# Kangfei/NNGP-src

Measured on AMD Instinct MI355X. Metric: NNGP kernel-build + GP-solve wall-clock (ms) and GFLOP/s at N train queries, higher is better.
Workload: dtype f32 (Cholesky products as split f16 x3, f32 accumulate; f64 build/CG/means; the posterior's float64-grade residual as exact int8 digit-plane products); 1 GPU; synthetic N=32768, d=128, 5-layer ReLU NNGP + full Cholesky posterior (configs[2], north-star target); N=32768, d=128, n_relu=3, get=nngp, M_test=1024, parallelism=single GPU

## Files before the change

nngp-src_amd/csrc/api.hip:

```cpp
#include "model.h"

namespace nngp {

static thread_local char g_err[1024] = "";

void set_error(const char* fmt, ...) {
    va_list ap;
    va_start(ap, fmt);
    vsnprintf(g_err, sizeof(g_err), fmt, ap);
    va_end(ap);
}

int make_arch_dev(const nngp_arch* arch, ArchDev* out) {
    NNGP_REQUIRE(arch != nullptr, "arch is NULL");
    NNGP_REQUIRE(arch->n_dense >= 1 && arch->n_dense <= NNGP_MAX_DENSE, "arch.n_dense must be in [1, %d] (got %d)",
                 NNGP_MAX_DENSE, arch->n_dense);
    out->n_dense = arch->n_dense;
    for (int l = 0; l < NNGP_MAX_DENSE; ++l) {
        out->w2[l] = l < arch->n_dense ? arch->w_std[l] * arch->w_std[l] : 0.0;
        out->b2[l] = l < arch->n_dense ? arch->b_std[l] * arch->b_std[l] : 0.0;
    }
    return 0;
}

// ... 205 lines not shown
    int rc = 0;
    m->arch = *arch;
    m->n_cap = n_cap; m->np_cap = round_up(n_cap, TB); m->m_cap = 0;
    m->ld = m->np_cap;
    m->d = d; m->ny = ny; m->get = get; m->diag_reg = diag_reg; m->absolute = diag_reg_absolute_scale;
    const int64_t np = m->np_cap;
    auto A = [&](int r) { if (rc == 0) rc = r; };
    A(dev_alloc(&m->x, n_cap * d)); A(dev_alloc(&m->y, n_cap * ny)); A(dev_alloc(&m->q, n_cap));
    A(dev_alloc(&m->kdiag, n_cap)); A(dev_alloc(&m->k64, np * np)); A(dev_alloc(&m->a32, np * np));
    A(dev_alloc(&m->dinv, (np / TB) * TB * TB)); A(dev_alloc(&m->clamped, 1)); A(dev_alloc(&m->alpha, n_cap * ny));
    A(dev_alloc(&m->pcg.r, np)); A(dev_alloc(&m->pcg.z, np)); A(dev_alloc(&m->pcg.p, np)); A(dev_alloc(&m->pcg.q, np));
    A(dev_alloc(&m->pcg.xcol, np)); A(dev_alloc(&m->pcg.bcol, np));
    A(dev_alloc(&m->pcg.f32a, np)); A(dev_alloc(&m->pcg.f32b, np)); A(dev_alloc(&m->pcg.f32c, np));
    A(dev_alloc(&m->pcg.scal, 32));
    A(dev_alloc(&m->pcg.symv_part, (np / TB) * np));
    A(dev_alloc(&m->pcg.dot_part, 32));
    A(dev_alloc(&m->pcg.dot_ctr, 1));
    if (rc == 0 && hipMemset(m->pcg.dot_ctr, 0, sizeof(unsigned)) != hipSuccess) rc = -1;
    m->pcg.symv_np = np;
    {
        const int64_t bs_cap = triinv_block(np);
        const int64_t nblk = (np + bs_cap - 1) / bs_cap;
        A(dev_alloc(&m->tri.tinv, nblk * bs_cap * bs_cap)); A(dev_alloc(&m->tri.xinv, nblk * bs_cap * bs_cap));
        A(dev_alloc(&m->tri.partial, (bs_cap / TB) * np)); A(dev_alloc(&m->tri.tmp, bs_cap));
    }
    if (rc == 0 && hipHostMalloc(reinterpret_cast<void**>(&m->pcg.host_scal), sizeof(double) * 32) != hipSuccess) {
        set_error("model_create: hipHostMalloc failed");
        rc = -1;
    }
    if (rc == 0) rc = lookahead_create(&m->la);
    int prio_least = 0, prio_greatest = 0;
    if (hipDeviceGetStreamPriorityRange(&prio_least, &prio_greatest) != hipSuccess) prio_least = prio_greatest = 0;
    if (rc == 0 && (hipStreamCreateWithPriority(&m->solve_stream, hipStreamNonBlocking, prio_greatest) != hipSuccess ||
                    hipEventCreateWithFlags(&m->ev_ready, hipEventDisableTiming) != hipSuccess ||
                    hipEventCreateWithFlags(&m->ev_lt, hipEventDisableTiming) != hipSuccess ||
                    hipEventCreateWithFlags(&m->ev_solved, hipEventDisableTiming) != hipSuccess ||
                    hipEventCreateWithFlags(&m->ev_predict, hipEventDisableTiming) != hipSuccess)) {
        set_error("model_create: could not create the solve stream");
        rc = -1;
    }
    if (rc == 0 && np >= 4 * kLookAheadNb) {
        m->split.rows_cap = np + 256;
        m->split.k_cap = kLookAheadNb;
        m->split.col_stride = m->split.rows_cap * m->split.k_cap * 4;
        const int64_t ncols = (np + kLookAheadNb - 1) / kLookAheadNb;
        rc = dev_alloc(&m->split.planes, ncols * m->split.col_stride);
        if (rc == 0) rc = dev_alloc(&m->split.counters, 16);
// ... 149 lines not shown
}

int nngp_model_factor_input_rows(nngp_model* m, int64_t row_begin, int64_t row_end, double shift_scale, void* stream) {
    hipStream_t s = (hipStream_t)stream;
    NNGP_REQUIRE(m != nullptr && m->built, "factor_input_rows: build the kernel rows first");
    NNGP_REQUIRE(0 <= row_begin && row_begin <= row_end && row_end <= m->n && shift_scale >= 1.0, "factor_input_rows: bad row range or shift");
    NNGP_TRY(drop_pending_solve(m));
    m->reg_fac = m->reg * shift_scale;
    m->k64_partial = true;
    return launch_factor_input(m->k64, m->ld, m->a32, m->ld, m->n, m->np, m->reg_fac, m->reg_fac + m->trace_mean, s, row_begin, row_end);
}

int nngp_model_factor_input_complete(nngp_model* m) {
    NNGP_REQUIRE(m != nullptr && m->built, "factor_input_complete: build the kernel rows first");
    NNGP_REQUIRE(m->k64_partial, "factor_input_complete: no rows of the factor input were converted (nngp_model_factor_input_rows) since the last build");
    m->a32_complete = true;
    return 0;
}

int nngp_model_precond(nngp_model* m, const double* r, double* z, void* stream) {
    NNGP_REQUIRE(m != nullptr && m->factored, "precond: factor first");
    NNGP_REQUIRE(r != nullptr && z != nullptr, "precond: NULL argument");
    NNGP_TRY(tri_join(m, (hipStream_t)stream));
    return precond_apply(m->a32, m->ld, m->tri, m->n, m->np, r, z, m->pcg, (hipStream_t)stream);
}

int nngp_model_matvec_rows(nngp_model* m, const double* p, double* q, int64_t row_begin, int64_t row_end, void* stream) {
    NNGP_REQUIRE(m != nullptr && m->built, "matvec_rows: build the kernel rows first");
    NNGP_REQUIRE(p != nullptr && q != nullptr && 0 <= row_begin && row_begin <= row_end && row_end <= m->n, "matvec_rows: bad arguments");
    return launch_gemv_f64(m->k64 + row_begin * m->ld, m->ld, row_end - row_begin, m->n, p, 1, q, 1, 0.0, (hipStream_t)stream);
}

int nngp_model_set_alpha(nngp_model* m, const double* alpha, int32_t iters, double rel_residual, void* stream) {
    hipStream_t s = (hipStream_t)stream;
    NNGP_REQUIRE(m != nullptr && m->factored && alpha != nullptr, "set_alpha: factor first");
    NNGP_TRY(drop_pending_solve(m));
    NNGP_HIP_CHECK(hipMemcpyAsync(m->alpha, alpha, sizeof(double) * m->n * m->ny, hipMemcpyDeviceToDevice, s));
    m->solved = true;
    m->solve_pending = false;
    m->cg_partial = false;
    m->have_alpha_event = false;
    m->iters = iters;
    m->relres = rel_residual;
    return 0;
}

int nngp_model_factor_end(nngp_model* m, void* stream) {
    hipStream_t s = (hipStream_t)stream;
    NNGP_REQUIRE(m != nullptr && m->built, "factor_end: build the kernel rows first");
    m->tri.bs = triinv_block(m->np);
    m->tri_stale = true;
    m->tri_pending = false;
    if (!m->split.l_ready && m->split.planes != nullptr && m->np >= 4 * m->split.k_cap && m->tri.bs % m->split.k_cap == 0 &&
        m->split.rows_cap >= m->np + 256) {
        const int64_t bs = m->split.k_cap, ldp = 4 * bs;
        for (int64_t j = 0, o = 0; o + bs < m->np; ++j, o += bs)
            NNGP_TRY(launch_split_rows(m->a32 + (o + bs) * m->ld + o, m->ld, m->np - o - bs, bs, m->split.scale,
                                       m->split.planes + j * m->split.col_stride + (o + bs) * ldp, ldp, s));
        m->split.l_ready = true;
    }
    m->factored = true;
    m->solved = false;
    m->lt_ready = false;
    return 0;
}

int nngp_model_factor_buffers(nngp_model* m, float** a32, int64_t* ld, float** dinv) {
    NNGP_REQUIRE(m != nullptr && m->have_train, "factor_buffers: call set_train first");
    if (a32) *a32 = m->a32;
    if (ld) *ld = m->ld;
    if (dinv) *dinv = m->dinv;
    return 0;
}

int nngp_model_factor(nngp_model* m, void* stream) {
// ... 49 lines not shown
    m->serving_ready = false;
    m->i8.k.ready = false;
    m->i8_checked = m->i8_distrusted = false;
    m->i8_guard_pending = false;
    BuildArgs a{};
    a.x1 = m->x; a.x2 = m->x; a.q1 = m->q; a.q2 = m->q;
    a.n1 = n1; a.n2 = n1; a.d = m->d;
    a.row_begin = n0; a.row_end = n1; a.sym = 0;
    a.ld64 = a.ld32 = m->ld;
    if (m->get == NNGP_GET_NNGP) a.nngp64 = m->k64; else a.ntk64 = m->k64;
    m->k64_symmetric = false;
    NNGP_TRY(launch_kernel_build(a, m->arch, s));
    NNGP_TRY(launch_mirror_rows_f64(m->k64, m->ld, n0, n1, s));
    NNGP_TRY(launch_zero_pad_f64(m->k64, m->ld, n1, np1, s));
    NNGP_TRY(launch_factor_input(m->k64, m->ld, m->a32, m->ld, n1, np1, m->reg_fac, m->reg_fac + m->trace_mean, s, r0));
    float* a10 = m->a32 + r0 * m->ld;
    NNGP_TRY(tri_join(m, s));
    NNGP_TRY(trsm_rlt_blocks_f32(a10, m->ld, rows, m->a32, m->ld, m->tri, r0, m->trsm_tmp, s));
    NNGP_TRY(launch_gemm_nt_f32(a10 + r0, m->ld, a10, m->ld, a10, m->ld, rows, rows, r0, -1.0f, 1.0f, true, s));
    NNGP_TRY(potrf_f32(a10 + r0, rows, m->ld, m->dinv + (r0 / TB) * TB * TB, m->clamped, (float)(0.25 * m->reg_fac), s));
    m->tri.bs = triinv_block(m->np);
    m->tri_stale = true;
    m->tri_pending = false;
    NNGP_TRY(tri_join(m, s));
    if (m->split.l_ready && m->split.scale == old_scale && m->split.rows_cap >= np1 + 256) {
        const int64_t bs = m->split.k_cap, ldp = 4 * bs;
        for (int64_t j = 0, o = 0; o + bs < np1; ++j, o += bs) {
            const int64_t first = (o + bs > r0) ? o + bs : r0;
            NNGP_TRY(launch_split_rows(m->a32 + first * m->ld + o, m->ld, np1 - first, bs, m->split.scale,
                                       m->split.planes + j * m->split.col_stride + first * ldp, ldp, s));
        }
    } else {
        m->split.l_ready = false;
    }
    m->split.lt_ready = false;
    m->lt_ready = false;
    m->aux_ready = false;
    (void)np0;
    return 0;
}

constexpr int kSolveAhead = 6;

constexpr double kPartialTol = 1e-6;

static void note_solve(nngp_model* m, int it, double rr) {
    int est = it;
    if (rr > m->pend_tol && rr > 0.0 && rr < 1.0 && it > 0) est = (int)ceil(it * log(m->pend_tol) / log(rr));
    if (est > m->iters) m->iters = est;
    if (rr > m->relres) m->relres = rr;
}

}
namespace nngp {
int run_pending_solve(nngp_model* m, hipStream_t user, bool order_user, bool allow_partial) {
    hipStream_t s = m->solve_stream;
    auto join_tri = [&]() -> int {
        NNGP_HIP_CHECK(hipStreamWaitEvent(s, m->ev_ready, 0));
        return tri_join(m, s);
    };
    if (!m->solve_pending) {
        if (!m->cg_partial || allow_partial) {
            if (order_user && m->solved && m->have_alpha_event) NNGP_HIP_CHECK(hipStreamWaitEvent(user, m->ev_solved, 0));
            return 0;
        }
        if (m->have_predict_event) NNGP_HIP_CHECK(hipStreamWaitEvent(s, m->ev_predict, 0));
        int it = 0;
        double rr = 0.0;
        NNGP_TRY(join_tri());
        NNGP_TRY(pcg_finish(m->k64, m->ld, m->n, m->reg, m->a32, m->ld, m->tri, m->np, m->pcg.xcol, m->pcg, m->cg_iters_done,
                            m->pend_max_iters, m->pend_tol, &it, &rr, s, true));
        NNGP_TRY(launch_strided_copy_f64(m->pcg.xcol, 1, m->alpha, m->ny, m->n, s));
        m->cg_partial = false;
        m->iters = 0;
        m->relres = 0.0;
        note_solve(m, it, rr);
        NNGP_HIP_CHECK(hipEventRecord(m->ev_solved, s));
        m->have_alpha_event = true;
        if (order_user) NNGP_HIP_CHECK(hipStreamWaitEvent(user, m->ev_solved, 0));
        else NNGP_HIP_CHECK(hipStreamSynchronize(s));
        return 0;
    }
// ... 30 lines not shown
            note_solve(m, it, rr);
        }
    }
    NNGP_HIP_CHECK(hipEventRecord(m->ev_solved, s));
    m->have_alpha_event = true;
    if (order_user) NNGP_HIP_CHECK(hipStreamWaitEvent(user, m->ev_solved, 0));
    else NNGP_HIP_CHECK(hipStreamSynchronize(s));
    return 0;
}

}

extern "C" {

int nngp_model_solve(nngp_model* m, int32_t max_iters, double tol, void* stream) {
    hipStream_t s = (hipStream_t)stream;
    NNGP_REQUIRE(m != nullptr && m->factored, "solve: factor first");
    NNGP_REQUIRE(!m->k64_partial, "solve: this model holds only its own kernel rows (row-sharded layout): the caller drives the CG "
                                  "(nngp_model_precond, nngp_model_matvec_rows) and hands alpha back with nngp_model_set_alpha");
    NNGP_TRY(drop_pending_solve(m));
    const double weak = (m->reg > 0.0 && m->reg_fac > m->reg) ? sqrt(m->reg_fac / m->reg) : 1.0;
    m->pend_max_iters = max_iters > 0 ? max_iters : (int)fmin(2000.0, 60.0 * weak);
    m->pend_tol = tol > 0.0 ? tol : 1e-10;
    NNGP_HIP_CHECK(hipEventRecord(m->ev_ready, s));
    m->solve_pending = true;
    m->solved = true;
    if (NNGP_KNOB(7) == 3) return run_pending_solve(m, s, true);
    if (NNGP_KNOB(0) & 32) return run_pending_solve(m, s, true, true);
    if (m->ny == 1 && NNGP_KNOB(0) == 64) {
        const int ahead = m->pend_max_iters < kSolveAhead ? m->pend_max_iters : kSolveAhead;
        NNGP_HIP_CHECK(hipStreamWaitEvent(m->solve_stream, m->ev_ready, 0));
        NNGP_TRY(tri_join(m, m->solve_stream));
        NNGP_TRY(launch_strided_copy_f64(m->y, 1, m->pcg.bcol, 1, m->n, m->solve_stream));
        NNGP_TRY(pcg_begin(m->k64, m->ld, m->n, m->reg, m->a32, m->ld, m->tri, m->np, m->pcg.bcol, m->pcg.xcol, m->pcg, ahead,
                           m->solve_stream));
        m->solve_ahead = ahead;
    }
    return 0;
}

int nngp_model_fit(nngp_model* m, const double* x, const double* y, int64_t n, void* stream) {
    NNGP_TRY(nngp_model_set_train(m, x, y, n, stream));
    NNGP_TRY(nngp_model_build_rows(m, 0, n, stream));
    NNGP_TRY(nngp_model_factor(m, stream));
    return nngp_model_solve(m, 0, 0.0, stream);
}

int nngp_model_kernel_buffer(nngp_model* m, double** k64, int64_t* ld) {
    NNGP_REQUIRE(m != nullptr && m->have_train, "kernel_buffer: call set_train first");
    if (k64) *k64 = m->k64;
    if (ld) *ld = m->ld;
    return 0;
}

int nngp_model_update_timer(nngp_model* m, int32_t enable) {
// ... 142 lines not shown
```

nngp-src_amd/csrc/api_predict.hip:

```cpp
#include "model.h"

namespace nngp {

int ensure_predict_capacity(nngp_model* m, int64_t mt, bool need_ktd) {
    if (mt > m->m_cap || m->b32 == nullptr) {
        const int64_t cap = mt > m->m_cap ? mt : m->m_cap;
        NNGP_HIP_CHECK(hipDeviceSynchronize());
        dev_free(m->xt_q); dev_free(m->tt_diag); dev_free(m->b32); dev_free(m->trsm_tmp);
        NNGP_TRY(dev_alloc(&m->xt_q, cap));
        NNGP_TRY(dev_alloc(&m->tt_diag, cap));
        NNGP_TRY(dev_alloc(&m->b32, round_up(cap, TB) * m->np_cap));
        NNGP_TRY(dev_alloc(&m->trsm_tmp, round_up(cap, TB) * triinv_block(m->np_cap)));
        if (m->split.planes != nullptr) {
            dev_free(m->split.planes_b); dev_free(m->split.row_inv);
            m->split.planes_b = nullptr; m->split.row_inv = nullptr;
            m->split.mb_cap = round_up(cap, TB);
            m->split.b_panels = (int)((triinv_block(m->np_cap) + m->split.k_cap - 1) / m->split.k_cap);
            NNGP_TRY(dev_alloc(&m->split.planes_b, (int64_t)(m->split.b_panels - 1) * m->split.col_stride + (m->split.mb_cap + 256) * m->split.k_cap * 4));
            NNGP_TRY(dev_alloc(&m->split.row_inv, m->split.mb_cap));
            tk_destroy(m->tk);
            m->tk = nullptr;
            if (m->split.k_cap == 1024 && triinv_block(m->np_cap) == 1024) NNGP_TRY(tk_create(&m->tk, m->np_cap, m->split.mb_cap) < 0 ? -1 : 0);
        }
        m->m_cap = cap;
// ... 254 lines not shown
    }
    NNGP_TRY(launch_gemm_nt_f64(out, np, rhs, np, z, np, m->k64, m->ld, mp, np, np, -1.0, 1.0, s));
    return launch_axpby_mat(out, 1.0, z, -m->reg, np, mp, np, s);
}

int tri_join(nngp_model* m, hipStream_t s) {
    if (m->tri_stale) {
        if (m->ev_tri == nullptr) NNGP_HIP_CHECK(hipEventCreateWithFlags(&m->ev_tri, hipEventDisableTiming));
        NNGP_TRY(triinv_build(m->a32, m->ld, m->dinv, m->np, m->tri, s));
        if (m->tk != nullptr && m->tri.bs == 1024) NNGP_TRY(tk_prepare_inverses(m->tk, m->tri, m->np, m->a32, m->ld, s));
        NNGP_HIP_CHECK(hipEventRecord(m->ev_tri, s));
        m->tri_stale = false;
        m->tri_pending = true;
        return 0;
    }
    if (m->tri_pending) NNGP_HIP_CHECK(hipStreamWaitEvent(s, m->ev_tri, 0));
    if (m->tk != nullptr && !tk_inverses_ready(m->tk) && m->tri.bs == 1024) {
        NNGP_TRY(tk_prepare_inverses(m->tk, m->tri, m->np, m->a32, m->ld, s));
        if (m->ev_tri == nullptr) NNGP_HIP_CHECK(hipEventCreateWithFlags(&m->ev_tri, hipEventDisableTiming));
        NNGP_HIP_CHECK(hipEventRecord(m->ev_tri, s));
        m->tri_pending = true;
    }
    return 0;
}

int tri_fork(nngp_model* m, hipStream_t s) {
    if (!m->tri_stale || m->la == nullptr || m->la->panel == nullptr || NNGP_KNOB(5) == 61) return 0;
    if (m->ev_tri == nullptr) NNGP_HIP_CHECK(hipEventCreateWithFlags(&m->ev_tri, hipEventDisableTiming));
    if (m->ev_tri_fork == nullptr) NNGP_HIP_CHECK(hipEventCreateWithFlags(&m->ev_tri_fork, hipEventDisableTiming));
    NNGP_HIP_CHECK(hipEventRecord(m->ev_tri_fork, s));
    NNGP_HIP_CHECK(hipStreamWaitEvent(m->la->panel, m->ev_tri_fork, 0));
    NNGP_TRY(triinv_build(m->a32, m->ld, m->dinv, m->np, m->tri, m->la->panel));
    if (m->tk != nullptr && m->tri.bs == 1024) NNGP_TRY(tk_prepare_inverses(m->tk, m->tri, m->np, m->a32, m->ld, m->la->panel));
    NNGP_HIP_CHECK(hipEventRecord(m->ev_tri, m->la->panel));
    m->tri_stale = false;
    m->tri_pending = true;
    return 0;
}

bool use_split_solves(const nngp_model* m, int64_t mp) {
    return m->split.l_ready && m->split.planes_b != nullptr && mp <= m->split.mb_cap && m->tri.bs % m->split.k_cap == 0 &&
           m->tri.bs / m->split.k_cap <= m->split.b_panels && m->tri.bs <= 2048 && NNGP_KNOB(7) == 0 && mp >= 256 && mp * m->np >= 7000000;
}

bool use_tickets(const nngp_model* m, int64_t mp) {
    return !m->tk_failed && m->tri.bs == 1024 && tk_usable(m->tk, mp, m->np) && NNGP_KNOB(9) != 16;
// ... 534 lines not shown
```

nngp-src_amd/csrc/common.h:

```cpp
#pragma once
#include <hip/hip_runtime.h>
#include <stdint.h>
#include <atomic>
#include <stdio.h>
#include <string.h>

#include "../../include/nngp_hip.h"
#include "../../include/nngp_rbf_gp.h"
#include "../../include/nngp_activations.h"
#include "../../include/nngp_mll.h"

namespace nngp {

constexpr int TB = 128;

void set_error(const char* fmt, ...);
void note_alloc();
#ifdef NNGP_TIMING_KNOBS
extern std::atomic<int> g_knobs[16];
#define NNGP_KNOB(i) (nngp::g_knobs[i].load(std::memory_order_relaxed))
#else
#define NNGP_KNOB(i) 0
#endif

// ... 207 lines not shown
struct I8Fuse {
    float* out32 = nullptr;
    int64_t ld32 = 0;
    double* part = nullptr;
};
int64_t i8s_col_blocks(int64_t cols);
int launch_i8s_combine(double* out, int64_t ldo, const double* cin, int64_t ldcin, double beta, double alpha, const double* g,
                       int64_t ldg, double gamma, const int32_t* partial, int64_t ldc, int64_t slab, int nchunk, int ndiag,
                       const double* sa, const double* sb, int64_t rows, int64_t cols, hipStream_t s, const I8Fuse* fuse = nullptr);
int launch_i8s_rowstat_finish(const double* part, int64_t cols, int64_t rows, const double* base, double* var, double* delta,
                              double* zstat, hipStream_t s);

int launch_gemm_nt_f64(double* c, int64_t ldc, const double* cin, int64_t ldcin, const double* a, int64_t lda,
                       const double* b, int64_t ldb, int64_t m, int64_t n, int64_t k, double alpha, double beta,
                       hipStream_t s, int kmode = 0);

int launch_transpose_blocks_f32(const float* src, float* dst, int64_t bs, int64_t count, hipStream_t s);
struct TriInv {
    int64_t bs = 0;
    float* tinv = nullptr;
    float* xinv = nullptr;
    float* partial = nullptr;
    float* tmp = nullptr;
    int64_t done_blocks = 0;
};
int64_t triinv_block(int64_t np);
int triinv_build(const float* l, int64_t ld, const float* dinv, int64_t np, TriInv& ti, hipStream_t s);
int triinv_build_range(const float* l, int64_t ld, const float* dinv, int64_t np, TriInv& ti, int64_t j0, int64_t j1, hipStream_t s);
int trsm_rlt_blocks_f32(float* b, int64_t ldb, int64_t m, const float* l, int64_t ld, const TriInv& ti, int64_t np,
                        float* tmp, hipStream_t s);
int trsm_rut_blocks_f32(float* b, int64_t ldb, int64_t m, const float* lt, int64_t ld, const TriInv& ti, int64_t np,
                        float* tmp, hipStream_t s);
int trsm_rlt_blocks_h3(float* b, int64_t ldb, int64_t m, const float* l, int64_t ld, const TriInv& ti, int64_t np,
                       float* tmp, const SplitWork& sw, hipStream_t s);
int trsm_rut_blocks_h3(float* b, int64_t ldb, int64_t m, const float* lt, int64_t ld, const TriInv& ti, int64_t np,
                       float* tmp, const SplitWork& sw, hipStream_t s);
int trsv_forward_f32(const float* l, int64_t ld, const TriInv& ti, int64_t np, float* b, float* x, hipStream_t s);
int trsv_backward_f32(const float* l, int64_t ld, const TriInv& ti, int64_t np, float* b, float* x, hipStream_t s);
struct TrsmTickets;
int tk_create(TrsmTickets** out, int64_t np_cap, int64_t m_cap);
void tk_destroy(TrsmTickets* tk);
int tk_prepare_inverses(TrsmTickets* tk, const TriInv& ti, int64_t np, const float* l, int64_t ld, hipStream_t s);
bool tk_inverses_ready(const TrsmTickets* tk);
void tk_invalidate_inverses(TrsmTickets* tk);
bool tk_usable(const TrsmTickets* tk, int64_t m, int64_t np);
int tk_solve(TrsmTickets* tk, float* b, int64_t ldb, int64_t m, int64_t np, const SplitWork& sw, bool backward, hipStream_t s, int reserve_cus = 0);
int tk_poll_error(TrsmTickets* tk, bool wait);
int tk_order_export(int mt, int nb, int tail_ct, int backward, int workers, int merged, int queues, int32_t* out, int32_t* queue_of, int64_t cap,
                    int64_t* count);
int launch_symv_f64(const double* a, int64_t lda, int64_t n, const double* x, double* y, double diag_add, double* part,
                    int64_t np, hipStream_t s);
int launch_gemv_f64(const double* a, int64_t lda, int64_t rows, int64_t cols, const double* x, int64_t incx,
                    double* y, int64_t incy, double diag_add, hipStream_t s);
struct PcgWork {
    double* r; double* z; double* p; double* q; double* xcol; double* bcol;
    float* f32a; float* f32b; float* f32c;
    double* dot_part = nullptr;
    unsigned* dot_ctr = nullptr;
    double* symv_part = nullptr;
    int64_t symv_np = 0;
    double* scal;
// ... 75 lines not shown
```

nngp-src_amd/csrc/model.h:

```cpp
#pragma once
#include <stdarg.h>
#include <stdlib.h>
#include <cmath>
#include <new>
#include <mutex>
#include "common.h"
#include <atomic>

namespace nngp {
extern std::atomic<long long> g_alloc_count;

template <typename T>
inline int dev_alloc(T** p, int64_t count) {
    *p = nullptr;
    if (count <= 0) return 0;
    NNGP_HIP_CHECK(hipMalloc(reinterpret_cast<void**>(p), sizeof(T) * (size_t)count));
    g_alloc_count.fetch_add(1, std::memory_order_relaxed);
    return 0;
}

template <typename T>
inline void dev_free(T*& p) {
    if (p) (void)hipFree(p);
    p = nullptr;
// ... 105 lines not shown
        hipEvent_t t0[kMax] = {}, t1[kMax] = {};
        double flops[kMax] = {};
    } trsm_t;
    hipEvent_t ev_tri = nullptr, ev_tri_fork = nullptr;
    hipEvent_t ev_ready = nullptr, ev_solved = nullptr;
    hipEvent_t ev_lt = nullptr;
    hipEvent_t ev_predict = nullptr;
    bool have_predict_event = false;
    bool solve_pending = false;
    bool cg_partial = false;
    bool have_alpha_event = false;
    int cg_iters_done = 0;
    int solve_ahead = 0;
    int pend_max_iters = 60;
    double pend_tol = 1e-10;

    ~nngp_model() {
        dev_free(x); dev_free(y); dev_free(q); dev_free(kdiag); dev_free(k64); dev_free(a32); dev_free(dinv);
        dev_free(clamped); dev_free(alpha);
        dev_free(pcg.r); dev_free(pcg.z); dev_free(pcg.p); dev_free(pcg.q); dev_free(pcg.xcol); dev_free(pcg.bcol);
        dev_free(pcg.f32a); dev_free(pcg.f32b); dev_free(pcg.f32c); dev_free(pcg.scal); dev_free(pcg.symv_part); dev_free(pcg.dot_part); dev_free(pcg.dot_ctr);
        if (pcg.host_scal) (void)hipHostFree(pcg.host_scal);
        if (pcg.iter_graph) (void)hipGraphExecDestroy(pcg.iter_graph);
        dev_free(tri.tinv); dev_free(tri.xinv); dev_free(tri.partial); dev_free(tri.tmp);
        lookahead_destroy(la);
        if (solve_stream) (void)hipStreamDestroy(solve_stream);
        if (ev_ready) (void)hipEventDestroy(ev_ready);
        if (ev_lt) (void)hipEventDestroy(ev_lt);
        if (ev_tri) (void)hipEventDestroy(ev_tri);
        for (int t = 0; t < TrsmTimer::kMax; ++t) { if (trsm_t.t0[t]) (void)hipEventDestroy(trsm_t.t0[t]); if (trsm_t.t1[t]) (void)hipEventDestroy(trsm_t.t1[t]); }
        if (ev_tri_fork) (void)hipEventDestroy(ev_tri_fork);
        if (ev_solved) (void)hipEventDestroy(ev_solved);
        if (ev_predict) (void)hipEventDestroy(ev_predict);
        if (ev_i8) (void)hipEventDestroy(ev_i8);
        if (ev_gate) (void)hipEventDestroy(ev_gate);
        dev_free(i8.k.planes); dev_free(i8.k.scale); dev_free(i8.aux.planes); dev_free(i8.aux.scale); dev_free(i8.zplanes);
        for (int t = 0; t < I8Work::kMaxTimed; ++t) { if (i8.t0[t]) (void)hipEventDestroy(i8.t0[t]); if (i8.t1[t]) (void)hipEventDestroy(i8.t1[t]); } dev_free(i8.zscale); dev_free(i8.partial); dev_free(i8.rowpart); dev_free(i8.counters);
        dev_free(split.planes); dev_free(split.counters); dev_free(split.planes_t); dev_free(split.planes_b); dev_free(split.row_inv);
        dev_free(split.ldiag); dev_free(split.dfrag); dev_free(split.dscale);
        tk_destroy(tk);
        dev_free(xt_q); dev_free(tt_diag); dev_free(ktd64); dev_free(b32); dev_free(trsm_tmp); dev_free(ktt64); dev_free(vvt32);
        dev_free(lt32); dev_free(dinvt); dev_free(z64); dev_free(r64); dev_free(covp64); dev_free(kaux64); dev_free(ktd_aux);
        dev_free(ainv64);
        dev_free(rows.p); dev_free(rows.q); dev_free(rows.rho); dev_free(rows.coef); dev_free(rows.tol); dev_free(rows.delta);
        dev_free(rows.var); dev_free(rows.state); dev_free(rows.live); dev_free(rows.zstat); dev_free(i8_guard);
        if (i8_guard_host) (void)hipHostFree(i8_guard_host);
        if (ev_guard) (void)hipEventDestroy(ev_guard);
// ... 1 lines not shown
    }
};


namespace nngp {
int ensure_predict_capacity(nngp_model* m, int64_t mt, bool need_ktd);
int ensure_full_cov_capacity(nngp_model* m, int64_t mt);
int drop_pending_solve(nngp_model* m);
void set_split_scale(nngp_model* m);
int ensure_refine_capacity(nngp_model* m, int64_t mp);
int ensure_lt_alloc(nngp_model* m);
int ensure_lt(nngp_model* m, hipStream_t s);
int ensure_lt_split(nngp_model* m, hipStream_t s);
bool use_i8s(const nngp_model* m, int64_t mp);
bool use_i8s_fine(const nngp_model* m, int64_t mp);
int i8s_planes_policy(const nngp_model* m);
int ensure_i8s(nngp_model* m, int64_t mp, I8Planes& pk, int planes);
int i8s_cut_planes(nngp_model* m, I8Planes& pk, const double* kmat, int64_t kld, hipStream_t s);
int i8s_product_rows(nngp_model* m, I8Planes& pk, const double* kmat, int64_t kld, double* out, const double* cin, double beta,
                     double alpha, double* z, double gamma, int64_t mp, hipStream_t s, int grade);
int residual_rows(nngp_model* m, double* out, const double* rhs, double* z, int64_t mp, hipStream_t s, bool first_residual);
int tri_join(nngp_model* m, hipStream_t s);
int tri_fork(nngp_model* m, hipStream_t s);
bool use_split_solves(const nngp_model* m, int64_t mp);
bool use_tickets(const nngp_model* m, int64_t mp);
bool cg_from_the_start(const nngp_model* m, int64_t mp);
int tickets_reserve(const nngp_model* m);
int tickets_check(nngp_model* m, bool wait);
int apply_forward_f32(nngp_model* m, int64_t mp, hipStream_t s);
int apply_inverse_f32(nngp_model* m, int64_t mp, hipStream_t s);
int refined_solve_rows(nngp_model* m, const double* rhs, int64_t mp, int sweeps, bool final_residual, hipStream_t s,
                       bool measure = false);
int rows_pcg_continue(nngp_model* m, int64_t mp, int max_iters, hipStream_t s);
int build_cross(nngp_model* m, const double* xt, const double* qt, int64_t mt, int64_t mp, bool nngp, double* out,
                hipStream_t s);
int run_pending_solve(nngp_model* m, hipStream_t user, bool order_user, bool allow_partial = false);
}
```

nngp-src_amd/csrc/solve.hip:

```cpp
#include "common.h"

namespace nngp {

namespace {

__global__ __launch_bounds__(256) void k_gemv_n_f32(const float* __restrict__ A, int64_t lda, int64_t rows,
                                                    int64_t cols, const float* __restrict__ x, float* y, int sub) {
    const int lane = threadIdx.x & 63;
    const int64_t row = (int64_t)blockIdx.x * 4 + (threadIdx.x >> 6);
    if (row >= rows) return;
    const float4* ar = reinterpret_cast<const float4*>(A + row * lda);
    const float4* xv = reinterpret_cast<const float4*>(x);
    float s = 0.0f;
    for (int64_t c = lane; c < cols / 4; c += 64) {
        const float4 a = ar[c], v = xv[c];
        s = fmaf(a.x, v.x, s);
        s = fmaf(a.y, v.y, s);
        s = fmaf(a.z, v.z, s);
        s = fmaf(a.w, v.w, s);
    }
#pragma unroll
    for (int off = 32; off > 0; off >>= 1) s += __shfl_xor(s, off);
    if (lane == 0) y[row] = sub ? y[row] - s : s;
}
// ... 1 lines not shown
__global__ __launch_bounds__(256) void k_gemv_t_partial_f32(const float* __restrict__ A, int64_t lda, int64_t cols,
                                                            const float* __restrict__ x, float* __restrict__ partial,
                                                            int64_t ldp) {
    __shared__ float xs[128];
    const int64_t r0 = (int64_t)blockIdx.y * 128;
    if (threadIdx.x < 128) xs[threadIdx.x] = x[r0 + threadIdx.x];
    __syncthreads();
    const int64_t c = (int64_t)blockIdx.x * 256 + threadIdx.x;
    if (c >= cols) return;
    const float* ap = A + r0 * lda + c;
    float s = 0.0f;
#pragma unroll 16
    for (int r = 0; r < 128; ++r) s = fmaf(ap[(int64_t)r * lda], xs[r], s);
    partial[(int64_t)blockIdx.y * ldp + c] = s;
}

__global__ __launch_bounds__(256) void k_sub_partials_f32(float* __restrict__ y, const float* __restrict__ partial,
                                                          int64_t ldp, int nchunk, int64_t cols) {
    const int64_t c = (int64_t)blockIdx.x * 256 + threadIdx.x;
    if (c >= cols) return;
    float s = 0.0f;
    for (int k = 0; k < nchunk; ++k) s += partial[(int64_t)k * ldp + c];
    y[c] -= s;
}

__global__ __launch_bounds__(256) void k_set_identity_blocks(float* __restrict__ t, int64_t bs, int64_t total) {
    const int64_t i = (int64_t)blockIdx.x * 256 + threadIdx.x;
    if (i >= total) return;
    const int64_t e = i % (bs * bs);
    t[i] = (e / bs == e % bs) ? 1.0f : 0.0f;
}

__global__ __launch_bounds__(256) void k_transpose_blocks(const float* __restrict__ src, float* __restrict__ dst,
                                                          int64_t bs) {
    __shared__ float tile[32][33];
    const int64_t base = (int64_t)blockIdx.z * bs * bs;
    const int tx = threadIdx.x & 31, ty = threadIdx.x >> 5;
    const int64_t c0 = (int64_t)blockIdx.x * 32, r0 = (int64_t)blockIdx.y * 32;
#pragma unroll
    for (int k = 0; k < 4; ++k) tile[ty + 8 * k][tx] = src[base + (r0 + ty + 8 * k) * bs + c0 + tx];
    __syncthreads();
#pragma unroll
    for (int k = 0; k < 4; ++k) dst[base + (c0 + ty + 8 * k) * bs + r0 + tx] = tile[tx][ty + 8 * k];
}

__global__ __launch_bounds__(256, 8) void k_symv_tiles_f64(const double* __restrict__ A, int64_t lda, int64_t n,
// ... 95 lines not shown
__global__ __launch_bounds__(256, 8) void k_dot(const double* __restrict__ a, const double* __restrict__ b, int64_t n,
                                                double* out, double* part, unsigned* counter) {
    __shared__ double red[4];
    __shared__ bool last;
    double s = 0.0;
    for (int64_t i = (int64_t)blockIdx.x * 256 + threadIdx.x; i < n; i += (int64_t)kDotBlocks * 256) s = fma(a[i], b[i], s);
    for (int off = 32; off > 0; off >>= 1) s += __shfl_down(s, off);
    if ((threadIdx.x & 63) == 0) red[threadIdx.x >> 6] = s;
    __syncthreads();
    if (threadIdx.x == 0) {
        part[blockIdx.x] = (red[0] + red[1]) + (red[2] + red[3]);
        __threadfence();
        last = atomicInc(counter, kDotBlocks - 1) == kDotBlocks - 1;
    }
    __syncthreads();
    if (last && threadIdx.x == 0) {
        __threadfence();
        double t = 0.0;
        for (int w = 0; w < kDotBlocks; ++w) t += __hip_atomic_load(&part[w], __ATOMIC_RELAXED, __HIP_MEMORY_SCOPE_AGENT);
        *out = t;
    }
}

__global__ void k_pcg_update_xr(double* x, double* r, const double* p, const double* q, int64_t n, const double* scal) {
    const int64_t i = (int64_t)blockIdx.x * 256 + threadIdx.x;
    if (i >= n) return;
    const double a = scal[1] != 0.0 ? scal[0] / scal[1] : 0.0;
    x[i] = fma(a, p[i], x[i]);
    r[i] = fma(-a, q[i], r[i]);
}

__global__ void k_pcg_update_p(double* p, const double* z, int64_t n, double* scal, int first) {
    const int64_t i = (int64_t)blockIdx.x * 256 + threadIdx.x;
    if (i >= n) return;
    if (first || scal[0] == 0.0) {
        p[i] = z[i];
    } else {
        p[i] = fma(scal[2] / scal[0], p[i], z[i]);
    }
}

__global__ void k_scal_shift(double* scal) { scal[0] = scal[2]; }

__global__ void k_f64_to_f32(const double* src, float* dst, int64_t n, int64_t np) {
    const int64_t i = (int64_t)blockIdx.x * 256 + threadIdx.x;
    if (i < np) dst[i] = i < n ? (float)src[i] : 0.0f;
}

__global__ void k_f32_to_f64(const float* src, double* dst, int64_t n) {
    const int64_t i = (int64_t)blockIdx.x * 256 + threadIdx.x;
// ... 173 lines not shown
}

int trsv_backward_f32(const float* l, int64_t ld, const TriInv& ti, int64_t np, float* b, float* x, hipStream_t s) {
    NNGP_REQUIRE(b != x, "trsv_backward: b and x must be different buffers");
    const int64_t bs = ti.bs;
    const int64_t nblk = (np + bs - 1) / bs;
    for (int64_t j = nblk - 1; j >= 0; --j) {
        const int64_t o = j * bs;
        const int64_t sz = (np - o < bs) ? np - o : bs;
        hipLaunchKernelGGL(k_gemv_n_f32, dim3((unsigned)((sz + 3) / 4)), dim3(256), 0, s, ti.tinv + j * bs * bs, bs, sz, sz,
                           b + o, x + o, 0);
        if (o > 0) {
            const int nchunk = (int)(sz / 128);
            hipLaunchKernelGGL(k_gemv_t_partial_f32, dim3((unsigned)((o + 255) / 256), (unsigned)nchunk), dim3(256), 0, s,
                               l + o * ld, ld, o, x + o, ti.partial, np);
            hipLaunchKernelGGL(k_sub_partials_f32, dim3((unsigned)((o + 255) / 256)), dim3(256), 0, s, b, ti.partial, np,
                               nchunk, o);
        }
    }
    NNGP_HIP_CHECK(hipGetLastError());
    return 0;
}

int launch_symv_f64(const double* a, int64_t lda, int64_t n, const double* x, double* y, double diag_add, double* part,
                    int64_t np, hipStream_t s) {
    if (n <= 0) return 0;
    NNGP_REQUIRE(part != nullptr && np % 128 == 0 && np >= n, "symv_f64: bad workspace");
    const int64_t nblk = (n + 127) / 128;
    hipLaunchKernelGGL(k_symv_tiles_f64, dim3((unsigned)(nblk * (nblk + 1) / 2)), dim3(256), 0, s, a, lda, n, x, part, np);
    hipLaunchKernelGGL(k_symv_reduce_f64, dim3(blocks256(n)), dim3(256), 0, s, part, nblk, np, n, x, diag_add, y);
    NNGP_HIP_CHECK(hipGetLastError());
    return 0;
}

int launch_gemv_f64(const double* a, int64_t lda, int64_t rows, int64_t cols, const double* x, int64_t incx,
                    double* y, int64_t incy, double diag_add, hipStream_t s) {
    if (rows <= 0) return 0;
    hipLaunchKernelGGL(k_gemv_f64, dim3((unsigned)rows), dim3(256), 0, s, a, lda, rows, cols, x, incx, y, incy,
                       diag_add);
    NNGP_HIP_CHECK(hipGetLastError());
    return 0;
}

namespace {
constexpr int kPcgHist = 8;
constexpr int kPcgMaxAhead = 22;

int pcg_iteration(const double* k64, int64_t ld, int64_t n, double reg, const float* l32, int64_t ld32, const TriInv& ti,
                  int64_t np, double* xcol, PcgWork& w, int it, double* rr_out, hipStream_t s) {
    hipLaunchKernelGGL(k_f64_to_f32, dim3(blocks256(np)), dim3(256), 0, s, w.r, w.f32a, n, np);
    NNGP_TRY(trsv_forward_f32(l32, ld32, ti, np, w.f32a, w.f32b, s));
    NNGP_TRY(trsv_backward_f32(l32, ld32, ti, np, w.f32b, w.f32c, s));
    hipLaunchKernelGGL(k_f32_to_f64, dim3(blocks256(n)), dim3(256), 0, s, w.f32c, w.z, n);
    hipLaunchKernelGGL(k_dot, dim3(kDotBlocks), dim3(256), 0, s, w.r, w.z, n, w.scal + 2, w.dot_part, w.dot_ctr);
    hipLaunchKernelGGL(k_pcg_update_p, dim3(blocks256(n)), dim3(256), 0, s, w.p, w.z, n, w.scal, it == 0);
    hipLaunchKernelGGL(k_scal_shift, dim3(1), dim3(1), 0, s, w.scal);
    if (w.symv_part != nullptr && w.symv_np >= np && n >= 4096 && NNGP_KNOB(5) != 7)
        NNGP_TRY(launch_symv_f64(k64, ld, n, w.p, w.q, reg, w.symv_part, w.symv_np, s));
    else
        NNGP_TRY(launch_gemv_f64(k64, ld, n, n, w.p, 1, w.q, 1, reg, s));
    hipLaunchKernelGGL(k_dot, dim3(kDotBlocks), dim3(256), 0, s, w.p, w.q, n, w.scal + 1, w.dot_part, w.dot_ctr);
    hipLaunchKernelGGL(k_pcg_update_xr, dim3(blocks256(n)), dim3(256), 0, s, xcol, w.r, w.p, w.q, n, w.scal);
    hipLaunchKernelGGL(k_dot, dim3(kDotBlocks), dim3(256), 0, s, w.r, w.r, n, rr_out, w.dot_part, w.dot_ctr);
    NNGP_HIP_CHECK(hipGetLastError());
    return 0;
}
}

int precond_apply(const float* l32, int64_t ld32, const TriInv& ti, int64_t n, int64_t np, const double* r, double* z, PcgWork& w,
                  hipStream_t s) {
    hipLaunchKernelGGL(k_f64_to_f32, dim3(blocks256(np)), dim3(256), 0, s, r, w.f32a, n, np);
    NNGP_TRY(trsv_forward_f32(l32, ld32, ti, np, w.f32a, w.f32b, s));
    NNGP_TRY(trsv_backward_f32(l32, ld32, ti, np, w.f32b, w.f32c, s));
    hipLaunchKernelGGL(k_f32_to_f64, dim3(blocks256(n)), dim3(256), 0, s, w.f32c, z, n);
    NNGP_HIP_CHECK(hipGetLastError());
    return 0;
}

int pcg_begin(const double* k64, int64_t ld, int64_t n, double reg, const float* l32, int64_t ld32, const TriInv& ti,
              int64_t np, const double* bcol, double* xcol, PcgWork& w, int ahead, hipStream_t s) {
    NNGP_REQUIRE(ahead >= 0 && ahead <= kPcgMaxAhead, "pcg_begin: at most %d iterations ahead", kPcgMaxAhead);
    NNGP_HIP_CHECK(hipMemsetAsync(xcol, 0, sizeof(double) * n, s));
    NNGP_HIP_CHECK(hipMemcpyAsync(w.r, bcol, sizeof(double) * n, hipMemcpyDeviceToDevice, s));
    hipLaunchKernelGGL(k_dot, dim3(kDotBlocks), dim3(256), 0, s, bcol, bcol, n, w.scal + kPcgHist, w.dot_part, w.dot_ctr);
    for (int it = 0; it < ahead; ++it)
        NNGP_TRY(pcg_iteration(k64, ld, n, reg, l32, ld32, ti, np, xcol, w, it, w.scal + kPcgHist + 1 + it, s));
    NNGP_HIP_CHECK(hipMemcpyAsync(w.host_scal + kPcgHist, w.scal + kPcgHist, sizeof(double) * (1 + ahead), hipMemcpyDeviceToHost, s));
    return 0;
}

int pcg_finish(const double* k64, int64_t ld, int64_t n, double reg, const float* l32, int64_t ld32, const TriInv& ti,
               int64_t np, double* xcol, PcgWork& w, int ahead, int max_iters, double tol, int* iters_out,
               double* relres_out, hipStream_t s, bool resume) {
// ... 75 lines not shown
```

Measured before the change: 168,000 GFLOP/s.

## Merge blocked triangular sweeps in PCG preconditioner using precomputed coupling blocks

Precomputes per-block coupling matrices (Xinv_{j+1}·L_{j+1,j} for the forward sweep, Tinv·L^T for the backward sweep) with batched GEMMs once after factorization. Each forward and backward block step then runs as a single fused kernel, and the f64<->f32 conversions and the scalar-shift kernel are folded into neighbouring kernels. The aim is fewer launches and serialized dependencies per PCG iteration. In exchange it costs two extra (nblk-1)·bs² float buffers, extra GEMM work per factorization, and some f32 reassociation in the preconditioner.

```diff
diff --git a/nngp-src_amd/csrc/api.hip b/nngp-src_amd/csrc/api.hip
--- a/nngp-src_amd/csrc/api.hip
+++ b/nngp-src_amd/csrc/api.hip
@@ -251,7 +251,10 @@
         const int64_t bs_cap = triinv_block(np);
         const int64_t nblk = (np + bs_cap - 1) / bs_cap;
         A(dev_alloc(&m->tri.tinv, nblk * bs_cap * bs_cap)); A(dev_alloc(&m->tri.xinv, nblk * bs_cap * bs_cap));
-        A(dev_alloc(&m->tri.partial, (bs_cap / TB) * np)); A(dev_alloc(&m->tri.tmp, bs_cap));
+        A(dev_alloc(&m->tri.partial, 2 * (bs_cap / TB) * np)); A(dev_alloc(&m->tri.tmp, bs_cap));
+        if (bs_cap == 1024 && nblk >= 2) {
+            A(dev_alloc(&m->tri.wf, (nblk - 1) * bs_cap * bs_cap)); A(dev_alloc(&m->tri.wb, (nblk - 1) * bs_cap * bs_cap));
+        }
     }
     if (rc == 0 && hipHostMalloc(reinterpret_cast<void**>(&m->pcg.host_scal), sizeof(double) * 32) != hipSuccess) {
         set_error("model_create: hipHostMalloc failed");
@@ -447,6 +450,7 @@
     NNGP_REQUIRE(m != nullptr && m->factored, "precond: factor first");
     NNGP_REQUIRE(r != nullptr && z != nullptr, "precond: NULL argument");
     NNGP_TRY(tri_join(m, (hipStream_t)stream));
+    NNGP_TRY(trw_join(m, (hipStream_t)stream));
     return precond_apply(m->a32, m->ld, m->tri, m->n, m->np, r, z, m->pcg, (hipStream_t)stream);
 }
 
@@ -476,6 +480,7 @@
     m->tri.bs = triinv_block(m->np);
     m->tri_stale = true;
     m->tri_pending = false;
+    m->tri.w_ready = false;
     if (!m->split.l_ready && m->split.planes != nullptr && m->np >= 4 * m->split.k_cap && m->tri.bs % m->split.k_cap == 0 &&
         m->split.rows_cap >= m->np + 256) {
         const int64_t bs = m->split.k_cap, ldp = 4 * bs;
@@ -571,6 +576,7 @@
     m->tri.bs = triinv_block(m->np);
     m->tri_stale = true;
     m->tri_pending = false;
+    m->tri.w_ready = false;
     NNGP_TRY(tri_join(m, s));
     if (m->split.l_ready && m->split.scale == old_scale && m->split.rows_cap >= np1 + 256) {
         const int64_t bs = m->split.k_cap, ldp = 4 * bs;
@@ -606,7 +612,8 @@
     hipStream_t s = m->solve_stream;
     auto join_tri = [&]() -> int {
         NNGP_HIP_CHECK(hipStreamWaitEvent(s, m->ev_ready, 0));
-        return tri_join(m, s);
+        NNGP_TRY(tri_join(m, s));
+        return trw_join(m, s);
     };
     if (!m->solve_pending) {
         if (!m->cg_partial || allow_partial) {
@@ -683,6 +690,10 @@
     const double weak = (m->reg > 0.0 && m->reg_fac > m->reg) ? sqrt(m->reg_fac / m->reg) : 1.0;
     m->pend_max_iters = max_iters > 0 ? max_iters : (int)fmin(2000.0, 60.0 * weak);
     m->pend_tol = tol > 0.0 ? tol : 1e-10;
+    if (!m->tri.w_ready && trsv_merged_applicable(m->tri, m->np) && NNGP_KNOB(15) != 1) {
+        NNGP_TRY(tri_join(m, s));
+        NNGP_TRY(trw_join(m, s));
+    }
     NNGP_HIP_CHECK(hipEventRecord(m->ev_ready, s));
     m->solve_pending = true;
     m->solved = true;
@@ -692,6 +703,7 @@
         const int ahead = m->pend_max_iters < kSolveAhead ? m->pend_max_iters : kSolveAhead;
         NNGP_HIP_CHECK(hipStreamWaitEvent(m->solve_stream, m->ev_ready, 0));
         NNGP_TRY(tri_join(m, m->solve_stream));
+        NNGP_TRY(trw_join(m, m->solve_stream));
         NNGP_TRY(launch_strided_copy_f64(m->y, 1, m->pcg.bcol, 1, m->n, m->solve_stream));
         NNGP_TRY(pcg_begin(m->k64, m->ld, m->n, m->reg, m->a32, m->ld, m->tri, m->np, m->pcg.bcol, m->pcg.xcol, m->pcg, ahead,
                            m->solve_stream));
diff --git a/nngp-src_amd/csrc/api_predict.hip b/nngp-src_amd/csrc/api_predict.hip
--- a/nngp-src_amd/csrc/api_predict.hip
+++ b/nngp-src_amd/csrc/api_predict.hip
@@ -300,6 +300,11 @@
         m->tri_pending = true;
     }
     return 0;
+}
+
+int trw_join(nngp_model* m, hipStream_t s) {
+    if (m->tri.w_ready || !trsv_merged_applicable(m->tri, m->np) || NNGP_KNOB(15) == 1) return 0;
+    return trsv_merged_build(m->a32, m->ld, m->np, m->tri, s);
 }
 
 int tri_fork(nngp_model* m, hipStream_t s) {
diff --git a/nngp-src_amd/csrc/common.h b/nngp-src_amd/csrc/common.h
--- a/nngp-src_amd/csrc/common.h
+++ b/nngp-src_amd/csrc/common.h
@@ -253,6 +253,9 @@
     float* xinv = nullptr;
     float* partial = nullptr;
     float* tmp = nullptr;
+    float* wf = nullptr;
+    float* wb = nullptr;
+    bool w_ready = false;
     int64_t done_blocks = 0;
 };
 int64_t triinv_block(int64_t np);
@@ -268,6 +271,8 @@
                        float* tmp, const SplitWork& sw, hipStream_t s);
 int trsv_forward_f32(const float* l, int64_t ld, const TriInv& ti, int64_t np, float* b, float* x, hipStream_t s);
 int trsv_backward_f32(const float* l, int64_t ld, const TriInv& ti, int64_t np, float* b, float* x, hipStream_t s);
+bool trsv_merged_applicable(const TriInv& ti, int64_t np);
+int trsv_merged_build(const float* l, int64_t ld, int64_t np, TriInv& ti, hipStream_t s);
 struct TrsmTickets;
 int tk_create(TrsmTickets** out, int64_t np_cap, int64_t m_cap);
 void tk_destroy(TrsmTickets* tk);
diff --git a/nngp-src_amd/csrc/model.h b/nngp-src_amd/csrc/model.h
--- a/nngp-src_amd/csrc/model.h
+++ b/nngp-src_amd/csrc/model.h
@@ -151,7 +151,7 @@
         dev_free(pcg.f32a); dev_free(pcg.f32b); dev_free(pcg.f32c); dev_free(pcg.scal); dev_free(pcg.symv_part); dev_free(pcg.dot_part); dev_free(pcg.dot_ctr);
         if (pcg.host_scal) (void)hipHostFree(pcg.host_scal);
         if (pcg.iter_graph) (void)hipGraphExecDestroy(pcg.iter_graph);
-        dev_free(tri.tinv); dev_free(tri.xinv); dev_free(tri.partial); dev_free(tri.tmp);
+        dev_free(tri.tinv); dev_free(tri.xinv); dev_free(tri.partial); dev_free(tri.tmp); dev_free(tri.wf); dev_free(tri.wb);
         lookahead_destroy(la);
         if (solve_stream) (void)hipStreamDestroy(solve_stream);
         if (ev_ready) (void)hipEventDestroy(ev_ready);
@@ -199,6 +199,7 @@
 int residual_rows(nngp_model* m, double* out, const double* rhs, double* z, int64_t mp, hipStream_t s, bool first_residual);
 int tri_join(nngp_model* m, hipStream_t s);
 int tri_fork(nngp_model* m, hipStream_t s);
+int trw_join(nngp_model* m, hipStream_t s);
 bool use_split_solves(const nngp_model* m, int64_t mp);
 bool use_tickets(const nngp_model* m, int64_t mp);
 bool cg_from_the_start(const nngp_model* m, int64_t mp);
diff --git a/nngp-src_amd/csrc/solve.hip b/nngp-src_amd/csrc/solve.hip
--- a/nngp-src_amd/csrc/solve.hip
+++ b/nngp-src_amd/csrc/solve.hip
@@ -47,6 +47,135 @@
     float s = 0.0f;
     for (int k = 0; k < nchunk; ++k) s += partial[(int64_t)k * ldp + c];
     y[c] -= s;
+}
+
+__device__ __forceinline__ float row_dot_f32(const float* __restrict__ arow, const float* xv, int c4n, int c4lo, int c4hi, int lane) {
+    const float4* ar = reinterpret_cast<const float4*>(arow);
+    const float4* xr = reinterpret_cast<const float4*>(xv);
+    float s = 0.0f;
+    for (int c = lane; c < c4n; c += 64) {
+        if (c < c4lo || c > c4hi) continue;
+        const float4 a = ar[c], v = xr[c];
+        s = fmaf(a.x, v.x, s);
+        s = fmaf(a.y, v.y, s);
+        s = fmaf(a.z, v.z, s);
+        s = fmaf(a.w, v.w, s);
+    }
+#pragma unroll
+    for (int off = 32; off > 0; off >>= 1) s += __shfl_xor(s, off);
+    return s;
+}
+
+__global__ __launch_bounds__(256) void k_trsv_fwd_first(const float* __restrict__ xinv, int64_t bs, int sz0, const double* __restrict__ r,
+                                                        int64_t n, int64_t np, float* __restrict__ b, float* __restrict__ x) {
+    __shared__ __attribute__((aligned(16))) float rs[1024];
+    const int nrow_wg = sz0 / 4;
+    if ((int)blockIdx.x >= nrow_wg) {
+        const int64_t i = (int64_t)sz0 + (int64_t)(blockIdx.x - nrow_wg) * 256 + threadIdx.x;
+        if (i < np) b[i] = i < n ? (float)r[i] : 0.0f;
+        return;
+    }
+    const int lane = threadIdx.x & 63, row0 = blockIdx.x * 4, row = row0 + (threadIdx.x >> 6);
+    for (int c = threadIdx.x; c < sz0; c += 256) rs[c] = (c <= row0 + 3 && c < n) ? (float)r[c] : 0.0f;
+    __syncthreads();
+    const float s = row_dot_f32(xinv + (int64_t)row * bs, rs, sz0 / 4, 0, row / 4, lane);
+    if (lane == 0) x[row] = s;
+}
+
+__global__ __launch_bounds__(256) void k_trsv_fwd_step(const float* __restrict__ lnext, int64_t ld, const float* __restrict__ xinv1,
+                                                       const float* __restrict__ w, int64_t bs, int sz1, int64_t rows,
+                                                       const float* __restrict__ xj, float* bnext, float* __restrict__ xnext) {
+    const int lane = threadIdx.x & 63;
+    const int64_t row = (int64_t)blockIdx.x * 4 + (threadIdx.x >> 6);
+    if (row >= rows) return;
+    const int c4 = (int)(bs / 4);
+    if (row < sz1) {
+        const float s1 = row_dot_f32(xinv1 + row * bs, bnext, sz1 / 4, 0, (int)row / 4, lane);
+        const float s2 = row_dot_f32(w + row * bs, xj, c4, 0, c4, lane);
+        if (lane == 0) xnext[row] = s1 - s2;
+    } else {
+        const float s = row_dot_f32(lnext + row * ld, xj, c4, 0, c4, lane);
+        if (lane == 0) bnext[row] -= s;
+    }
+}
+
+__global__ __launch_bounds__(256) void k_trsv_bwd_first(const float* __restrict__ tinv, int64_t bs, int sz, const float* __restrict__ b,
+                                                        float* __restrict__ x, double* __restrict__ z, int64_t o, int64_t n) {
+    const int lane = threadIdx.x & 63, row = blockIdx.x * 4 + (threadIdx.x >> 6);
+    if (row >= sz) return;
+    const float s = row_dot_f32(tinv + (int64_t)row * bs, b, sz / 4, row / 4, sz / 4, lane);
+    if (lane == 0) {
+        x[row] = s;
+        if (o + row < n) z[row] = (double)s;
+    }
+}
+
+__global__ __launch_bounds__(256) void k_trsv_bwd_step(const float* __restrict__ lj, int64_t ld, const float* __restrict__ tprev,
+                                                       const float* __restrict__ w, int64_t bs, int sz, int64_t o, const float* __restrict__ xj,
+                                                       float* b, float* __restrict__ x, double* __restrict__ z, int64_t n,
+                                                       const float* __restrict__ pprev, int nprev, float* __restrict__ pcur, int64_t ldp) {
+    __shared__ __attribute__((aligned(16))) float bu[1024];
+    const int nrow_wg = (int)(bs / 4);
+    const int64_t op = o - bs;
+    if ((int)blockIdx.x < nrow_wg) {
+        const int lane = threadIdx.x & 63, row0 = blockIdx.x * 4, row = row0 + (threadIdx.x >> 6);
+        for (int c = threadIdx.x; c < (int)bs; c += 256) {
+            float v = 0.0f;
+            if (c >= row0) {
+                float t = 0.0f;
+                for (int k = 0; k < nprev; ++k) t += pprev[(int64_t)k * ldp + op + c];
+                v = b[op + c] - t;
+            }
+            bu[c] = v;
+        }
+        __syncthreads();
+        const int c4 = (int)(bs / 4);
+        const float s1 = row_dot_f32(tprev + (int64_t)row * bs, bu, c4, row / 4, c4, lane);
+        const float s2 = row_dot_f32(w + (int64_t)row * bs, xj, sz / 4, 0, c4, lane);
+        if (lane == 0) {
+            const float v = s1 - s2;
+            x[op + row] = v;
+            if (op + row < n) z[op + row] = (double)v;
+        }
+        return;
+    }
+    float* xs = bu;
+    const int64_t ncb = op / 256;
+    const int64_t q = (int64_t)blockIdx.x - nrow_wg;
+    const int chunk = (int)(q / ncb);
+    const int64_t c = (q % ncb) * 256 + threadIdx.x;
+    if (chunk >= sz / 128) return;
+    if (threadIdx.x < 128) xs[threadIdx.x] = xj[chunk * 128 + threadIdx.x];
+    __syncthreads();
+    const float* ap = lj + (int64_t)chunk * 128 * ld + c;
+    float s = 0.0f;
+#pragma unroll 16
+    for (int r = 0; r < 128; ++r) s = fmaf(ap[(int64_t)r * ld], xs[r], s);
+    pcur[(int64_t)chunk * ldp + c] = s;
+    if (chunk == 0 && nprev > 0) {
+        float t = 0.0f;
+        for (int k = 0; k < nprev; ++k) t += pprev[(int64_t)k * ldp + c];
+        b[c] -= t;
+    }
+}
+
+__global__ __launch_bounds__(256) void k_transpose_strided_blocks(const float* __restrict__ src, int64_t lds, int64_t sstride,
+                                                                  float* __restrict__ dst, int64_t bs, int rows_last) {
+    __shared__ float tile[32][33];
+    const int64_t blk = blockIdx.z;
+    const float* sp = src + blk * sstride;
+    float* dp = dst + blk * bs * bs;
+    const int tx = threadIdx.x & 31, ty = threadIdx.x >> 5;
+    const int64_t c0 = (int64_t)blockIdx.x * 32, r0 = (int64_t)blockIdx.y * 32;
+    const int64_t nvalid = (blk == (int64_t)gridDim.z - 1) ? rows_last : bs;
+#pragma unroll
+    for (int k = 0; k < 4; ++k) {
+        const int64_t r = r0 + ty + 8 * k;
+        tile[ty + 8 * k][tx] = r < nvalid ? sp[r * lds + c0 + tx] : 0.0f;
+    }
+    __syncthreads();
+#pragma unroll
+    for (int k = 0; k < 4; ++k) dp[(c0 + ty + 8 * k) * bs + r0 + tx] = tile[tx][ty + 8 * k];
 }
 
 __global__ __launch_bounds__(256) void k_set_identity_blocks(float* __restrict__ t, int64_t bs, int64_t total) {
@@ -188,10 +317,12 @@
     }
 }
 
-__global__ void k_pcg_update_xr(double* x, double* r, const double* p, const double* q, int64_t n, const double* scal) {
+__global__ void k_pcg_update_xr(double* x, double* r, const double* p, const double* q, int64_t n, double* scal, int shift) {
     const int64_t i = (int64_t)blockIdx.x * 256 + threadIdx.x;
     if (i >= n) return;
-    const double a = scal[1] != 0.0 ? scal[0] / scal[1] : 0.0;
+    const double rz = shift ? scal[2] : scal[0];
+    if (shift && i == 0) scal[0] = rz;
+    const double a = scal[1] != 0.0 ? rz / scal[1] : 0.0;
     x[i] = fma(a, p[i], x[i]);
     r[i] = fma(-a, q[i], r[i]);
 }
@@ -411,6 +542,67 @@
     return 0;
 }
 
+bool trsv_merged_applicable(const TriInv& ti, int64_t np) {
+    return ti.bs == 1024 && np >= 2 * ti.bs && np % TB == 0 && ti.wf != nullptr && ti.wb != nullptr;
+}
+
+int trsv_merged_build(const float* l, int64_t ld, int64_t np, TriInv& ti, hipStream_t s) {
+    NNGP_REQUIRE(trsv_merged_applicable(ti, np), "trsv_merged_build: not applicable");
+    const int64_t bs = ti.bs, blk = bs * bs, nb = (np + bs - 1) / bs, tail = np - (nb - 1) * bs;
+    const int full = (int)(tail == bs ? nb - 1 : nb - 2);
+    const float* sub = l + bs * ld;
+    hipLaunchKernelGGL(k_transpose_strided_blocks, dim3((unsigned)(bs / 32), (unsigned)(bs / 32), (unsigned)(nb - 1)), dim3(256), 0, s, sub, ld,
+                       bs * ld + bs, ti.wb, bs, (int)tail);
+    NNGP_HIP_CHECK(hipGetLastError());
+    if (full > 0)
+        NNGP_TRY(launch_gemm_nt_f32_batched(ti.wf, bs, ti.xinv + blk, bs, ti.wb, bs, bs, bs, bs, 1.0f, 0.0f, false, full, blk, blk, blk, s));
+    if (full < nb - 1)
+        NNGP_TRY(launch_gemm_nt_f32(ti.wf + (nb - 2) * blk, bs, ti.xinv + (nb - 1) * blk, bs, ti.wb + (nb - 2) * blk, bs, tail, bs, tail, 1.0f,
+                                    0.0f, false, s));
+    if (full > 0)
+        NNGP_TRY(launch_gemm_nt_f32_batched(ti.wb, bs, ti.tinv, bs, sub, ld, bs, bs, bs, 1.0f, 0.0f, false, full, blk, blk, bs * ld + bs, s));
+    if (full < nb - 1)
+        NNGP_TRY(launch_gemm_nt_f32(ti.wb + (nb - 2) * blk, bs, ti.tinv + (nb - 2) * blk, bs, sub + (nb - 2) * (bs * ld + bs), ld, bs, tail, bs,
+                                    1.0f, 0.0f, false, s));
+    ti.w_ready = true;
+    return 0;
+}
+
+static int trsv_forward_merged(const float* l, int64_t ld, const TriInv& ti, int64_t n, int64_t np, const double* r, float* bw, float* x,
+                               hipStream_t s) {
+    const int64_t bs = ti.bs, blk = bs * bs, nb = (np + bs - 1) / bs;
+    hipLaunchKernelGGL(k_trsv_fwd_first, dim3((unsigned)(bs / 4 + (np - bs + 255) / 256)), dim3(256), 0, s, ti.xinv, bs, (int)bs, r, n, np, bw, x);
+    for (int64_t j = 0; j + 1 < nb; ++j) {
+        const int64_t o1 = (j + 1) * bs, rows = np - o1, sz1 = rows < bs ? rows : bs;
+        hipLaunchKernelGGL(k_trsv_fwd_step, dim3((unsigned)((rows + 3) / 4)), dim3(256), 0, s, l + o1 * ld + j * bs, ld, ti.xinv + (j + 1) * blk,
+                           ti.wf + j * blk, bs, (int)sz1, rows, x + j * bs, bw + o1, x + o1);
+    }
+    NNGP_HIP_CHECK(hipGetLastError());
+    return 0;
+}
+
+static int trsv_backward_merged(const float* l, int64_t ld, const TriInv& ti, int64_t n, int64_t np, float* b, float* x, double* z,
+                                hipStream_t s) {
+    const int64_t bs = ti.bs, blk = bs * bs, nb = (np + bs - 1) / bs;
+    const int64_t ol = (nb - 1) * bs, szl = np - ol;
+    hipLaunchKernelGGL(k_trsv_bwd_first, dim3((unsigned)(szl / 4)), dim3(256), 0, s, ti.tinv + (nb - 1) * blk, bs, (int)szl, b + ol, x + ol, z + ol,
+                       ol, n);
+    float* part[2] = {ti.partial, ti.partial + (bs / TB) * np};
+    int nprev = 0;
+    for (int64_t j = nb - 1; j >= 1; --j) {
+        const int64_t o = j * bs, sz = (np - o < bs) ? np - o : bs;
+        const int nchunk = (int)(sz / 128);
+        const int64_t grid = bs / 4 + ((o - bs) / 256) * nchunk;
+        hipLaunchKernelGGL(k_trsv_bwd_step, dim3((unsigned)grid), dim3(256), 0, s, l + o * ld, ld, ti.tinv + (j - 1) * blk, ti.wb + (j - 1) * blk, bs,
+                           (int)sz, o, x + o, b, x, z, n, part[(j + 1) & 1], nprev, part[j & 1], np);
+        nprev = nchunk;
+    }
+    NNGP_HIP_CHECK(hipGetLastError());
+    return 0;
+}
+
+static bool use_merged_sweeps(const TriInv& ti, int64_t np) { return ti.w_ready && trsv_merged_applicable(ti, np) && NNGP_KNOB(15) != 1; }
+
 int launch_symv_f64(const double* a, int64_t lda, int64_t n, const double* x, double* y, double diag_add, double* part,
                     int64_t np, hipStream_t s) {
     if (n <= 0) return 0;
@@ -437,19 +629,17 @@
 
 int pcg_iteration(const double* k64, int64_t ld, int64_t n, double reg, const float* l32, int64_t ld32, const TriInv& ti,
                   int64_t np, double* xcol, PcgWork& w, int it, double* rr_out, hipStream_t s) {
-    hipLaunchKernelGGL(k_f64_to_f32, dim3(blocks256(np)), dim3(256), 0, s, w.r, w.f32a, n, np);
-    NNGP_TRY(trsv_forward_f32(l32, ld32, ti, np, w.f32a, w.f32b, s));
-    NNGP_TRY(trsv_backward_f32(l32, ld32, ti, np, w.f32b, w.f32c, s));
-    hipLaunchKernelGGL(k_f32_to_f64, dim3(blocks256(n)), dim3(256), 0, s, w.f32c, w.z, n);
+    const bool merged = use_merged_sweeps(ti, np);
+    NNGP_TRY(precond_apply(l32, ld32, ti, n, np, w.r, w.z, w, s));
     hipLaunchKernelGGL(k_dot, dim3(kDotBlocks), dim3(256), 0, s, w.r, w.z, n, w.scal + 2, w.dot_part, w.dot_ctr);
     hipLaunchKernelGGL(k_pcg_update_p, dim3(blocks256(n)), dim3(256), 0, s, w.p, w.z, n, w.scal, it == 0);
-    hipLaunchKernelGGL(k_scal_shift, dim3(1), dim3(1), 0, s, w.scal);
+    if (!merged) hipLaunchKernelGGL(k_scal_shift, dim3(1), dim3(1), 0, s, w.scal);
     if (w.symv_part != nullptr && w.symv_np >= np && n >= 4096 && NNGP_KNOB(5) != 7)
         NNGP_TRY(launch_symv_f64(k64, ld, n, w.p, w.q, reg, w.symv_part, w.symv_np, s));
     else
         NNGP_TRY(launch_gemv_f64(k64, ld, n, n, w.p, 1, w.q, 1, reg, s));
     hipLaunchKernelGGL(k_dot, dim3(kDotBlocks), dim3(256), 0, s, w.p, w.q, n, w.scal + 1, w.dot_part, w.dot_ctr);
-    hipLaunchKernelGGL(k_pcg_update_xr, dim3(blocks256(n)), dim3(256), 0, s, xcol, w.r, w.p, w.q, n, w.scal);
+    hipLaunchKernelGGL(k_pcg_update_xr, dim3(blocks256(n)), dim3(256), 0, s, xcol, w.r, w.p, w.q, n, w.scal, merged ? 1 : 0);
     hipLaunchKernelGGL(k_dot, dim3(kDotBlocks), dim3(256), 0, s, w.r, w.r, n, rr_out, w.dot_part, w.dot_ctr);
     NNGP_HIP_CHECK(hipGetLastError());
     return 0;
@@ -458,6 +648,10 @@
 
 int precond_apply(const float* l32, int64_t ld32, const TriInv& ti, int64_t n, int64_t np, const double* r, double* z, PcgWork& w,
                   hipStream_t s) {
+    if (use_merged_sweeps(ti, np)) {
+        NNGP_TRY(trsv_forward_merged(l32, ld32, ti, n, np, r, w.f32a, w.f32b, s));
+        return trsv_backward_merged(l32, ld32, ti, n, np, w.f32b, w.f32c, z, s);
+    }
     hipLaunchKernelGGL(k_f64_to_f32, dim3(blocks256(np)), dim3(256), 0, s, r, w.f32a, n, np);
     NNGP_TRY(trsv_forward_f32(l32, ld32, ti, np, w.f32a, w.f32b, s));
     NNGP_TRY(trsv_backward_f32(l32, ld32, ti, np, w.f32b, w.f32c, s));
```

After: 164,800 GFLOP/s, median of 2. -2.0%, worse.
